# OpenVisualCloud/SVT-VP9

Hardware: AMD Instinct MI355X
Metric: hot-path frames/sec (+ Mpixels/sec): block-level DSP path (picture analysis + ME + inter prediction from reconstructed references + DCT/quant/recon + deblock + reference padding), 3840x2160p60 yuv420p enc-mode 8; no mode decision, no entropy coding -- not encoded frames (higher is better)
Workload: dtype u8

## Files before the change

### include/svtvp9_hip.h

```cpp
#ifndef SVTVP9_HIP_H
#define SVTVP9_HIP_H

#include <stddef.h>
#include <stdint.h>

#ifdef __cplusplus
extern "C" {
#endif

typedef enum svt_hip_status {
    SVT_HIP_OK                 = 0,
    SVT_HIP_ERR_BAD_PARAMETER  = -1,
    SVT_HIP_ERR_NO_RESOURCES   = -2,
    SVT_HIP_ERR_DEVICE         = -3,
    SVT_HIP_ERR_UNSUPPORTED    = -4
} svt_hip_status;

typedef struct svt_hip_ctx svt_hip_ctx;


#define SVT_ME_PU_COUNT 85
#define SVT_SB_SIZE 64

typedef struct svt_plane {
// ... 52 lines not shown

typedef struct svt_me_pu_result {
    int16_t         x_mv_l0, y_mv_l0, x_mv_l1, y_mv_l1;
    svt_me_dist_dir distortion_direction[3];
    uint8_t         total_me_candidate_index;
    uint8_t         pad_[7];
} svt_me_pu_result;

int32_t svt_hip_sb_count(int32_t pic_width, int32_t pic_height);

int32_t svt_hip_input_resolution(int32_t pic_width, int32_t pic_height);

typedef struct svt_me_picture_config {
    int32_t pic_width, pic_height;
    int32_t enc_mode;
    int32_t tune;
    int32_t frame_rate;
    int32_t num_ref_lists;
    int32_t temporal_layer_index;
    int32_t hierarchical_levels;
    int32_t is_used_as_reference;
    int32_t same_ref_poc;
    int32_t rate_control_mode;
} svt_me_picture_config;

int32_t svt_hip_me_params_derive(svt_me_params *p, const svt_me_picture_config *cfg);

int32_t svt_hip_me_params_preset(svt_me_params *p, int32_t pic_width, int32_t pic_height, int32_t enc_mode,
                                 int32_t tune, int32_t num_ref_lists, int32_t temporal_layer_index,
                                 int32_t hierarchical_levels);

int32_t svt_hip_me_kernel_instance(const svt_me_params *p);
int32_t svt_hip_me_last_instance(const svt_hip_ctx *ctx);
int32_t svt_hip_me_lds_bytes(const svt_me_params *p, int32_t compact);
int32_t svt_hip_ctx_set_intra_workgroups(svt_hip_ctx *ctx, int32_t n);
int32_t svt_hip_ctx_warm(svt_hip_ctx *ctx);
int32_t svt_hip_ctx_warm_scratch(svt_hip_ctx *ctx, int32_t scratch_bytes);
int32_t svt_hip_me_params_same_launch(const svt_me_params *a, const svt_me_params *b);

int32_t svt_hip_ctx_create(svt_hip_ctx **ctx, int32_t device_ordinal);
int32_t svt_hip_ctx_create_on_stream(svt_hip_ctx **ctx, int32_t device_ordinal, void *hip_stream);
int32_t svt_hip_ctx_create_cu_mask(svt_hip_ctx **ctx, int32_t device, const uint32_t *cu_mask, int32_t mask_words);
void *svt_hip_ctx_stream(svt_hip_ctx *ctx);
void    svt_hip_ctx_destroy(svt_hip_ctx *ctx);
int32_t svt_hip_ctx_synchronize(svt_hip_ctx *ctx);
const char *svt_hip_last_error(void);
float   svt_hip_last_kernel_ms(svt_hip_ctx *ctx);

int32_t svt_hip_mem_alloc(svt_hip_ctx *ctx, size_t bytes, void **d_ptr);
void    svt_hip_mem_free(svt_hip_ctx *ctx, void *d_ptr);
int32_t svt_hip_mem_upload_2d(svt_hip_ctx *ctx, void *d_dst, size_t dst_stride, const void *src, size_t src_stride, size_t width_bytes,
                              size_t rows);
int32_t svt_hip_mem_download(svt_hip_ctx *ctx, void *dst, const void *d_src, size_t bytes);
int32_t svt_hip_mem_upload_2d_async(svt_hip_ctx *ctx, void *d_dst, size_t dst_stride, const void *src, size_t src_stride, size_t width_bytes,
                                    size_t rows);
int32_t svt_hip_mem_upload_planes_async(svt_hip_ctx *ctx, int32_t n_planes, void *const *d_dst, const size_t *dst_stride, const void *const *src,
                                        const size_t *src_stride, const size_t *width_bytes, const size_t *rows);
int32_t svt_hip_mem_upload_2d_direct(svt_hip_ctx *ctx, void *d_dst, size_t dst_stride, const void *src, size_t src_stride, size_t width_bytes,
                                     size_t rows);
int32_t svt_hip_mem_upload_wait(svt_hip_ctx *ctx);
void    svt_hip_host_unregister_all(void);
void    svt_hip_host_registry_retain(void);
void    svt_hip_host_registry_release(void);
int32_t svt_hip_ctx_marker_record(svt_hip_ctx *ctx, uint64_t *marker);
int32_t svt_hip_ctx_marker_query(svt_hip_ctx *ctx, uint64_t marker);
int32_t svt_hip_ctx_marker_wait(svt_hip_ctx *ctx, uint64_t marker);
// ... 484 lines not shown
```

### svt-vp9_amd/binding.py

```python
import ctypes as C
import os

import numpy as np

HERE = os.path.dirname(os.path.abspath(__file__))
LIB_PATH = os.environ.get("SVT_HIP_LIB") or os.path.join(HERE, "libsvtvp9_hip.so")

SVT_ME_PU_COUNT = 85


class Plane(C.Structure):
    _fields_ = [("buf", C.c_void_p), ("stride", C.c_int32), ("origin_x", C.c_int32), ("origin_y", C.c_int32),
                ("width", C.c_int32), ("height", C.c_int32)]


class PaPicture(C.Structure):
    _fields_ = [("full", Plane), ("quarter", Plane), ("sixteenth", Plane)]


class MeParams(C.Structure):
    _fields_ = [(n, C.c_uint8) for n in (
        "num_ref_lists", "temporal_layer_index", "hierarchical_levels", "enable_hme_flag",
        "enable_hme_level_0_flag", "enable_hme_level_1_flag", "enable_hme_level_2_flag", "cu8x8_mode",
        "cu16x16_mode", "same_ref_poc", "rate_control_mode", "fractional_search_method",
# ... 138 lines not shown
MODES_TABLES_DTYPE = np.dtype([("kf_y_mode_prob", "u1", (10, 10, 9)), ("kf_uv_mode_prob", "u1", (10, 9)), ("kf_partition_probs", "u1", (16, 3)), ("skip_probs", "u1", (3,))])
assert MODES_TABLES_DTYPE.itemsize == 900 + 90 + 48 + 3
MODES_BAD_GRID = 0xFFFFFFFF
MODES_UNIT_BOOLS = 48


class ModesPicture(C.Structure):
    _fields_ = [("d_lf_mi", C.c_void_p), ("d_eob_map", C.c_void_p), ("d_tok_off", C.c_void_p), ("d_bools", C.c_void_p), ("d_segments", C.c_void_p),
                ("d_n_bools", C.c_void_p), ("capacity", C.c_uint32), ("pad_", C.c_uint32)]

OIS_BLOCK_DTYPE = np.dtype([("sad", "<u4"), ("uv_sad", "<u4"), ("mode", "u1"), ("uv_mode", "u1"), ("pad", "u1", (2,))])
assert OIS_BLOCK_DTYPE.itemsize == 12
OIS_PER_SB = 340
OIS_NONE = 0xFFFFFFFF

EXPORTS = [
    "svt_hip_sb_count", "svt_hip_input_resolution", "svt_hip_me_params_derive", "svt_hip_me_params_preset", "svt_hip_ctx_create", "svt_hip_ctx_create_on_stream", "svt_hip_ctx_create_cu_mask", "svt_hip_ctx_stream",
    "svt_hip_ctx_destroy", "svt_hip_ctx_synchronize", "svt_hip_last_error", "svt_hip_last_kernel_ms",
    "svt_hip_mem_alloc", "svt_hip_mem_free", "svt_hip_mem_upload_2d", "svt_hip_mem_upload_2d_async", "svt_hip_mem_upload_planes_async", "svt_hip_mem_download", "svt_hip_mem_set",
    "svt_hip_ctx_marker_record", "svt_hip_ctx_marker_query", "svt_hip_ctx_marker_wait", "svt_hip_minigop_split",
    "svt_hip_me_picture_device", "svt_hip_me_batch_device", "svt_hip_me_batch_layers_device", "svt_hip_me_picture", "svt_hip_sad_loop_batch_device",
    "svt_hip_me_zz_sad_device", "svt_hip_me_similar_collocated", "svt_hip_me_sb_stats_device", "svt_hip_pa_prepare_batch_device", "svt_hip_pa_mean_variance_device",
    "svt_hip_quant_tables_init", "svt_hip_tq_batch_device", "svt_hip_tq_batch_dist_device", "svt_hip_tq_rd_batch_device", "svt_hip_tq_rd_batch_multi_device", "svt_hip_rate_scan4x4_table", "svt_hip_tq_batch", "svt_hip_lf_thresh_init", "svt_hip_lf_level_from_q",
    "svt_hip_lf_frame_device", "svt_hip_lf_batch_device", "svt_hip_lf_frame", "svt_hip_lf_build_masks",
    "svt_hip_inter_pred_batch_device", "svt_hip_inter_pred_frame", "svt_hip_ref_pad_batch_device", "svt_hip_coeff_rate_batch_device", "svt_hip_coeff_rate_batch",
    "svt_hip_gop_owner", "svt_hip_gop_assign", "svt_hip_minigop_reference_source", "svt_hip_device_set_create", "svt_hip_device_set_size",
    "svt_hip_device_set_ctx", "svt_hip_device_set_destroy", "svt_hip_ref_handoff_device",
    "svt_ivf_stream_header", "svt_ivf_packetize",
    "svt_hip_tq_blocks_from_grid", "svt_hip_vp9_iscan_tables", "svt_hip_vp9_qindex_from_qp", "svt_hip_vp9_dc_step", "svt_hip_vp9_ac_step",
    "svt_hip_quant_tables_for_qindex", "svt_hip_encdec_flags_derive", "svt_hip_encdec_work_create", "svt_hip_encdec_work_destroy",
    "svt_hip_encdec_batch_device", "svt_hip_encdec_intra_device", "svt_hip_md_intra_default_device", "svt_hip_encdec_work_status", "svt_hip_encdec_work_download", "svt_hip_md_default_batch_device",
    "svt_hip_md_default_picture", "svt_hip_lf_build_masks_device", "svt_hip_ctx_wait_marker", "svt_hip_host_alloc", "svt_hip_host_free",
    "svt_hip_mem_download_2d_async", "svt_hip_mem_copy_2d_device", "svt_hip_encdec_work_set_stage_hook", "svt_hip_me_params_same_launch", "svt_hip_me_kernel_instance", "svt_hip_ctx_set_intra_workgroups", "svt_hip_ctx_warm", "svt_hip_ctx_warm_scratch", "svt_hip_lf_reserve",
    "svt_hip_me_last_instance", "svt_hip_me_lds_bytes", "svt_hip_vp9_layer_qindex", "svt_hip_mem_upload_2d_direct", "svt_hip_mem_upload_wait", "svt_hip_host_unregister_all", "svt_hip_host_registry_retain", "svt_hip_host_registry_release",
    "svt_hip_intra_search_device", "svt_hip_md_intra_search_device", "svt_hip_md_intra_search_picture",
    "svt_hip_pa_noise_params_derive", "svt_hip_pa_noise_batch_device", "svt_hip_pa_histogram_batch_device", "svt_hip_pa_chroma_mean_batch_device",
    "svt_hip_vp9_scan_tables", "svt_hip_tokenize_blocks_device", "svt_hip_tokenize_blocks", "svt_hip_tokenize_blocks_host", "svt_hip_tokenize_batch_device", "svt_hip_tokenize_picture",
    "svt_hip_tokenize_capacity",
    "svt_hip_boolcode_set_tables", "svt_hip_boolcode_batch_device", "svt_hip_boolcode", "svt_hip_boolcode_host", "svt_hip_boolcode_capacity", "svt_hip_boolcode_bools_capacity",
    "svt_hip_boolcode_geometry",
    "svt_hip_modes_set_tables", "svt_hip_modes_kf_batch_device", "svt_hip_modes_kf_picture", "svt_hip_modes_segments", "svt_hip_modes_bools_capacity",
]

_lib = None


def load():
    global _lib
    if _lib is None:
        if not os.path.exists(LIB_PATH):
            raise RuntimeError(f"{LIB_PATH} not built: run `python -c 'import __graft_entry__ as g; g.build()'`")
        try:
            import torch
        except Exception:
            pass
        _lib = C.CDLL(LIB_PATH)
        _lib.svt_hip_last_error.restype = C.c_char_p
        _lib.svt_hip_ctx_stream.restype = C.c_void_p
        _lib.svt_hip_ctx_stream.argtypes = [C.c_void_p]
        _lib.svt_hip_last_kernel_ms.restype = C.c_float
        _lib.svt_hip_last_kernel_ms.argtypes = [C.c_void_p]
        _lib.svt_hip_lf_thresh_init.restype = None
        _lib.svt_hip_vp9_iscan_tables.restype = C.POINTER(C.c_int16)
        _lib.svt_hip_vp9_iscan_tables.argtypes = [C.POINTER(C.POINTER(C.c_uint32)), C.POINTER(C.c_int32)]
        _lib.svt_hip_vp9_scan_tables.restype = C.POINTER(C.c_int16)
        _lib.svt_hip_vp9_scan_tables.argtypes = [C.POINTER(C.POINTER(C.c_uint32)), C.POINTER(C.c_int32)]
        _lib.svt_hip_tokenize_capacity.restype = C.c_uint32
# ... 64 lines not shown
```

### svt-vp9_amd/csrc/me_fast.h

```cpp
#ifndef SVT_ME_FAST_H
#define SVT_ME_FAST_H
#include "me_core.h"

#ifndef SVT_HOST_EMU

constexpr bool me_fast_params_ok(uint8_t hme, uint8_t l0, uint8_t l1, uint8_t l2, uint8_t single, uint8_t method, uint8_t model, uint8_t f64,
                                 uint8_t cu16, uint8_t cu8) {
    return hme && l0 && !l1 && !l2 && single && method == SVT_SUB_SAD_SEARCH && model == 1 && !f64 && cu16 == 0 && cu8 == 1;
}

#define FME_ACC(st, s) ((uint32_t *)(st)->hme_sad + 5 * (s))
#define FME_HKEY(st, l) ((uint32_t *)(st)->hme_keys + (l))
#define FME_GATE(st) (&(st)->supel[0])
#define FME_QTAB(st) ((uint32_t *)(st)->spu)
#define FME_BTAB(st) ((uint32_t *)(st)->spu + 32)
SVT_DEV uint32_t fme_src_code(const me_ctx_t *c, int plane, int dx, int dy) {
    return plane == ME_PF ? (0x8000u | (uint32_t)(128 + ME_MUL(dy, c->L.region_stride) + dx))
                          : (uint32_t)(128 + ME_MUL(plane - 1, c->L.plane_bytes) + ME_MUL(dy, c->L.plane_stride) + dx);
}

SVT_DEV uint32_t fme_wave_sum63(uint32_t v) {
    v = svt_row_prefix_add(v, 16);
    v += (uint32_t)__builtin_amdgcn_update_dpp(0, (int)v, 0x142, 0xa, 0xf, false);
    v += (uint32_t)__builtin_amdgcn_update_dpp(0, (int)v, 0x143, 0xc, 0xf, false);
// ... 83 lines not shown
        uint32_t        lo = q[0];
        _Pragma("unroll") for (int i = 0; i < 8; i++) {
            const uint32_t hi = q[i + 1];
            acc = svt_sad4(svt_alignbyte(hi, lo, sh), sp[i], acc);
            lo = hi;
        }
    }
    acc = fme_wave_sum63(acc);
    if (tid == 63) slot[0] = acc;
}

SVT_DEV void fph_load_rect(int tid, uint8_t *dst, int dst_stride, const uint8_t *src, int src_stride, int nd, int rows) {
    const int      nu = (nd + 3) >> 2, n = nu * rows, last = 4 * nd - 16;
    const uint32_t inv = me_magics.v[nu];
    for (int t0 = tid; t0 < n; t0 += 2 * SVT_NT) {
        me_u32x4 v[2];
        int      o[2];
        _Pragma("unroll") for (int u = 0; u < 2; u++) {
            const int t = t0 + u * SVT_NT;
            o[u] = -1;
            if (t < n) {
                const int r = inv ? (int)__umulhi((uint32_t)t, inv) : t, i = t - ME_MUL(r, nu);
                const int b = 16 * i < last ? 16 * i : last;
                v[u] = me_ld128u_g(src + (uint32_t)(ME_MUL(r, src_stride) + b));
                o[u] = ME_MUL(r, dst_stride) + b;
            }
        }
        _Pragma("unroll") for (int u = 0; u < 2; u++)
            if (o[u] >= 0) {
                uint32_t *d = (uint32_t *)(dst + o[u]);
                d[0] = v[u].x; d[1] = v[u].y; d[2] = v[u].z; d[3] = v[u].w;
            }
    }
}

template <int WS> SVT_DEV void fph_hme_search(const me_ctx_t *c, int tid, int ws_rt, int sw, int nr, int y0, uint32_t *key) {
    const int      ws = WS ? WS : ws_rt, ng2 = sw >> 3, ntask = ME_MUL(ng2, nr);
    const uint32_t inv = me_magics.v[ng2];
    uint32_t       b0 = 0xffffffffu, b1 = 0xffffffffu, b2 = 0xffffffffu, b3 = 0xffffffffu;
    const uint32_t *blk = (const uint32_t *)c->st->sixteenth_sb;
    const bool tile32 = ng2 == 8;
    const int  nt = tile32 ? ((nr + 31) & ~31) * 8 : ntask;
    for (int T = tid; T < nt; T += SVT_NT) {
        int y, g;
        if (tile32) {
            const int l = T & 63, blk32 = T >> 8, wv = (T >> 6) & 3;
            y = 32 * blk32 + 4 * wv + ((l >> 3) & 1) + 2 * ((l >> 5) & 1) + 16 * ((l >> 4) & 1);
            g = 2 * (l & 7);
            if (y >= nr) continue;
        } else {
            y = (int)__umulhi((uint32_t)T, inv); g = 2 * (T - ME_MUL(y, ng2));
        }
        uint32_t o0 = (uint32_t)(c->planes - c->lds) + (uint32_t)(ME_MUL(y, ws) + 4 * g), o1 = o0 + 4, o2 = o0 + 12 * ws, o3 = o2 + 4;
        __asm__("" : "+v"(o0));
        __asm__("" : "+v"(o1));
        __asm__("" : "+v"(o2));
        __asm__("" : "+v"(o3));
        uint64_t acc0 = 0, acc1 = 0, acc2 = 0, acc3 = 0;
        _Pragma("unroll") for (int j = 0; j < 8; j++) {
            const uint8_t *wa = c->lds + (j < 6 ? o0 + 2 * j * ws : o2 + 2 * (j - 6) * ws), *wb = c->lds + (j < 6 ? o1 + 2 * j * ws : o3 + 2 * (j - 6) * ws);
            const uint64_t p0 = *(const me_u64a4 *)wa, p1 = *(const me_u64a4 *)wb, p2 = *(const me_u64a4 *)(wa + 8), p3 = *(const me_u64a4 *)(wb + 8),
                           p4 = *(const me_u64a4 *)(wa + 16);
            const uint32_t s0 = blk[4 * j], s1 = blk[4 * j + 1], s2 = blk[4 * j + 2], s3 = blk[4 * j + 3];
            uint64_t       a = (j & 1) ? acc1 : acc0, e = (j & 1) ? acc3 : acc2;
            a = svt_qsad(p0, s0, a); e = svt_qsad(p1, s0, e);
            a = svt_qsad(p1, s1, a); e = svt_qsad(p2, s1, e);
// ... 349 lines not shown
                uint32_t s[5];
                fme_center_sums(FME_ACC(st, 2 * list + 1), 2, s);
                z = s[0] << 1; hh = s[1] << 1;
            }
            if (z <= hh) { xsc = 0; ysc = 0; loaded = 0; }
        }
        FME_MARK(3);
        if (!loaded) {
            FME_SET_AREA();
            FME_LOAD_REGION();
        }
#undef FME_SET_AREA
#undef FME_LOAD_REGION
        FME_MARK(4);
        {
            uint32_t *U = (uint32_t *)c->planes;
            if (saw >= 8 && (saw & 7) == 0 && saw * sah <= 4096) {
                ME_PHASE(ph_fullpel_fused(c, tid, saw, sah, 0));
                FME_MARK(5);
                FME_MARK(6);
            } else {
                const int max_pos = c->L.scratch_bytes / (4 * ME_PU_STRIDE);
                int       rows_chunk = max_pos / saw;
                if (rows_chunk < 1) rows_chunk = 1;
                if (rows_chunk > sah) rows_chunk = sah;
                for (int y0 = 0; y0 < sah; y0 += rows_chunk) {
                    const int ny = y0 + rows_chunk <= sah ? rows_chunk : sah - y0;
                    ME_PHASE(ph_fullpel_sad8(c, tid, U, saw, y0, ny, w8));
                    ME_PHASE(ph_fullpel_sum16(c, tid, U, saw, ny, w8));
                    ME_PHASE(ph_fullpel_sum32(c, tid, U, ny * saw));
                    ME_PHASE(ph_fullpel_argmin(c, tid, U, saw, y0, ny));
                }
            }
            ME_PHASE(fph_decode_gate(c, tid, list, saw, sox, soy); ph_interp_strips(c, tid, W, H));
        }
        FME_MARK(7);
        const uint32_t gate = (uint32_t)ME_UNI(*FME_GATE(st));
        const int      en32 = (int)(gate & 1u), en16 = (int)((gate >> 1) & 1u);
        FME_MARK(8);
        FME_MARK(9);
        const int fast_bi = nlist == 2;
        if (en32 || en16 || fast_bi) ME_PHASE(fph_subpel(c, tid, list, sox, soy, en32, en16, fast_bi, pred0_regs));
        FME_MARK(10);
        FME_MARK(11);
        FME_MARK(12);
    }

    uint32_t *ow = (uint32_t *)c->planes;
    ME_PHASE(ph_output(c, tid, 0, ow));
    {
        uint32_t SVT_GLOBAL *g = SVT_AS_GLOBAL(uint32_t, c->pic->results + (size_t)c->sb_index * 85);
        for (int t = tid; t < 850; t += SVT_NT) g[t] = ow[t];
        if (c->pic->rcme && tid == 0) {
            uint32_t acc = 0;
            for (int i = 0; i < 16; i++) acc += ow[(5 + i) * 10 + 2];
            *SVT_AS_GLOBAL(uint32_t, &c->pic->rcme[c->sb_index]) = acc;
        }
    }
    FME_MARK(13);
}

#endif
#endif
```

### svt-vp9_amd/csrc/me_kernel.hip

```cpp
#include <hip/hip_runtime.h>
#include "me_core.h"
#include "me_fast.h"
#include "me_layout.h"
#include "me_spec.h"
#include "svt_ctx.h"
#include <stdio.h>
#include <stdlib.h>

extern __shared__ __align__(16) uint8_t svt_lds[];

#ifndef ME_WAVES_PER_EU
#define ME_WAVES_PER_EU 3
#endif
#ifndef ME_WAVES_PER_EU_SPEC
#define ME_WAVES_PER_EU_SPEC 5
#endif
template <int SPEC, bool FAST, bool COMPACT = false>
__device__ __forceinline__ void me_kernel_body(const me_pic_dev *__restrict__ pics, svt_me_params p, me_lds_layout L, int n_sb, int nx, int pic_w, int pic_h,
                                               int total, int chunk, unsigned long long *prof, uint32_t *redo = nullptr) {
    const int b = blockIdx.x, j = b >> 3;
    const int pic = j / chunk, sb = (b & 7) * chunk + (j - pic * chunk);
    if (sb >= n_sb || pic * n_sb >= total) return;
    if (!COMPACT && redo && !redo[pic * n_sb + sb]) return;
    me_ctx_t  c;
    c.redo = COMPACT ? redo + pic * n_sb + sb : nullptr;
    c.pic = &pics[pic];
    svt_me_params pp = p;
    pp.num_ref_lists = c.pic->num_ref_lists; pp.temporal_layer_index = c.pic->temporal_layer_index;
    pp.hierarchical_levels = c.pic->hierarchical_levels; pp.same_ref_poc = c.pic->same_ref_poc;
    L.hme_w0[0] = c.pic->hme_w0[0]; L.hme_w0[1] = c.pic->hme_w0[1]; L.hme_h0[0] = c.pic->hme_h0[0]; L.hme_h0[1] = c.pic->hme_h0[1];
    L.hme_tw0 = c.pic->hme_tw0; L.hme_th0 = c.pic->hme_th0;
    if constexpr (SPEC != 0) me_spec_apply<SPEC>(&pp);
    c.p   = &pp;
    if constexpr (SPEC != 0) {
        me_lds_layout G = L;
        me_lds_layout_geom_ex(&pp, &G, COMPACT);
        L.region_stride = G.region_stride; L.plane_stride = G.plane_stride; L.plane_bytes = G.plane_bytes; L.region_rows = G.region_rows;
        L.cand_dwords = G.cand_dwords; L.scratch_bytes = G.scratch_bytes;
        L.off_state = G.off_state; L.off_src = G.off_src; L.off_region = G.off_region; L.off_planes = G.off_planes;
        L.off_quarter = G.off_quarter; L.off_ssd = G.off_ssd; L.off_cand = G.off_cand; L.off_cand_hi = G.off_cand_hi; L.off_pred0 = G.off_pred0;
// ... 98 lines not shown
    static_assert(me_spec_fast(S), "me_fast.h does not serve this specialisation");
    return me_launch_kernel(svt_me_fast_kernel<S>, a, L);
}
template <int S> static hipError_t me_dispatch_sb(const me_launch_args &a, const me_lds_layout &L, const me_lds_layout &Lc, uint32_t *d_redo) {
    if constexpr (me_spec_has_compact(S))
        if (d_redo) {
            const hipError_t e = me_launch_kernel(svt_me_sb_kernel<S, true>, a, Lc, d_redo);
            return e != hipSuccess ? e : me_launch_kernel(svt_me_sb_kernel<S, false>, a, L, d_redo);
        }
    return me_launch_kernel(svt_me_sb_kernel<S, false>, a, L, (uint32_t *)nullptr);
}

static int32_t me_launch(svt_hip_ctx *ctx, int32_t n_pics, const svt_pa_picture *cur, const svt_pa_picture *ref0, const svt_pa_picture *ref1,
                         const svt_me_params *params_all, int params_stride, svt_me_pu_result *const *d_results, uint32_t *const *d_rcme) {
    if (!ctx || !cur || !ref0 || !params_all || !d_results || n_pics < 1) return svt_set_error(SVT_HIP_ERR_BAD_PARAMETER, "me: null argument");
    const svt_me_params *params = params_all;
    for (int i = 0; i < (params_stride ? n_pics : 1); i++) {
        const svt_me_params *q = &params_all[i];
        if (q->num_ref_lists < 1 || q->num_ref_lists > 2) return svt_set_error(SVT_HIP_ERR_BAD_PARAMETER, "me: num_ref_lists");
        if (q->num_ref_lists == 2 && !ref1) return svt_set_error(SVT_HIP_ERR_BAD_PARAMETER, "me: ref1 missing for B picture");
        if (q->hierarchical_levels > 5 || q->temporal_layer_index > 5 || q->number_hme_search_region_in_width > 2 ||
            q->number_hme_search_region_in_height > 2)
            return svt_set_error(SVT_HIP_ERR_BAD_PARAMETER, "me: parameter out of range");
        if (q->search_area_width < 1 || q->search_area_height < 1) return svt_set_error(SVT_HIP_ERR_BAD_PARAMETER, "me: empty full-pel search area");
        if (i && !me_params_same_config(params, q))
            return svt_set_error(SVT_HIP_ERR_BAD_PARAMETER, "me: the pictures of one launch may differ in num_ref_lists, temporal_layer_index, hierarchical_levels and same_ref_poc only");
    }
    me_lds_layout L;
    if (me_lds_layout_compute(params, &L)) return svt_set_error(SVT_HIP_ERR_UNSUPPORTED, "me: search area does not fit in LDS");
    const int W = cur[0].full.width, H = cur[0].full.height;
    if (W < 64 || H < 64 || (W & 7) || (H & 7)) return svt_set_error(SVT_HIP_ERR_BAD_PARAMETER, "me: picture size");
    const int nx = (W + 63) / 64, ny = (H + 63) / 64, n_sb = nx * ny;
    HIP_TRY(hipSetDevice(ctx->device));
    me_pic_dev *h = nullptr, *d = nullptr;
    if (svt_ctx_stage(ctx, sizeof(me_pic_dev) * (size_t)n_pics, (void **)&h, (void **)&d)) return svt_set_error(SVT_HIP_ERR_NO_RESOURCES, "me: descriptor buffers");
    bool fast_ok = (W & 63) == 0;
    for (int i = 0; i < n_pics; i++) {
        if (cur[i].full.width != W || cur[i].full.height != H) return svt_set_error(SVT_HIP_ERR_BAD_PARAMETER, "me: batch pictures differ in size");
        memset(&h[i], 0, sizeof h[i]);
        h[i].cur    = cur[i];
        h[i].ref[0] = ref0[i];
        if (ref1) h[i].ref[1] = ref1[i];
        h[i].results = d_results[i];
        h[i].rcme    = d_rcme ? d_rcme[i] : nullptr;
        const svt_me_params *q = &params_all[params_stride ? i : 0];
        me_lds_layout        Li;
        if (me_lds_layout_compute(q, &Li)) return svt_set_error(SVT_HIP_ERR_UNSUPPORTED, "me: search area does not fit in LDS");
        h[i].num_ref_lists = q->num_ref_lists; h[i].temporal_layer_index = q->temporal_layer_index;
        h[i].hierarchical_levels = q->hierarchical_levels; h[i].same_ref_poc = q->same_ref_poc;
        h[i].hme_w0[0] = Li.hme_w0[0]; h[i].hme_w0[1] = Li.hme_w0[1]; h[i].hme_h0[0] = Li.hme_h0[0]; h[i].hme_h0[1] = Li.hme_h0[1];
        h[i].hme_tw0 = Li.hme_tw0; h[i].hme_th0 = Li.hme_th0;
        {
            const int wbytes = Li.hme_tw0 + 16 + 3;
            int       ws = ((wbytes + 3) & ~3) + 4;
            if (((ws >> 2) & 1) == 0) ws += 4;
            const int band = Li.scratch_bytes / ws - 14;
            h[i].hme_band = (int16_t)(band > 256 ? 256 : band);
            if (band < 1 || Li.hme_tw0 > 256 || Li.hme_th0 > 256) fast_ok = false;
        }
    }
    HIP_TRY(hipMemcpyAsync(d, h, sizeof(me_pic_dev) * (size_t)n_pics, hipMemcpyHostToDevice, ctx->stream));
    const int total = n_sb * n_pics, chunk = (n_sb + 7) / 8;
    static const bool want_prof = getenv("SVT_HIP_ME_PROFILE") != nullptr;
    unsigned long long *d_prof = nullptr;
    if (want_prof) {
        d_prof = (unsigned long long *)svt_ctx_slot(ctx, 25, 32 * sizeof(unsigned long long));
        if (d_prof) HIP_TRY(hipMemsetAsync(d_prof, 0, 32 * sizeof(unsigned long long), ctx->stream));
    }
#ifdef ME_FINE_PROF
    { const char *sa = getenv("SVT_HIP_ME_STOP"); int v = sa ? atoi(sa) : -1; HIP_TRY(hipMemcpyToSymbolAsync(HIP_SYMBOL(g_me_stop_after), &v, sizeof v, 0, hipMemcpyHostToDevice, ctx->stream)); }
#endif
    static const bool no_spec = getenv("SVT_HIP_ME_GENERIC") != nullptr;
    static const bool no_fast = getenv("SVT_HIP_ME_NOFAST") != nullptr;
    const int spec = no_spec ? 0 : me_spec_match(params);
    me_lds_layout Lc = L;
    uint32_t     *d_redo = nullptr;
    if (me_spec_has_compact(spec) && (params->search_area_width & 7) == 0 && params->search_area_width <= 127 && me_lds_layout_compute_ex(params, &Lc, 1) == 0 &&
        me_lds_workgroups_per_cu(&Lc) > me_lds_workgroups_per_cu(&L)) {
        d_redo = (uint32_t *)svt_ctx_slot(ctx, 39, (size_t)total * sizeof(uint32_t));
        if (!d_redo) return svt_set_error(SVT_HIP_ERR_NO_RESOURCES, "me: redo flags");
        HIP_TRY(hipMemsetAsync(d_redo, 0, (size_t)total * sizeof(uint32_t), ctx->stream));
    }
    HIP_TRY(hipEventRecord(ctx->ev_start, ctx->stream));
    const bool           fast = fast_ok && !no_fast && me_spec_fast(spec);
    const me_launch_args a = {ctx->stream, chunk * 8 * n_pics, d, params, n_sb, nx, W, H, total, chunk, d_prof};
    switch (spec) {
    case 1: HIP_TRY(fast ? me_dispatch_fast<1>(a, L) : me_dispatch_sb<1>(a, L, Lc, d_redo)); break;
    case 2: HIP_TRY(me_dispatch_sb<2>(a, L, Lc, d_redo)); break;
    case 3: HIP_TRY(me_dispatch_sb<3>(a, L, Lc, d_redo)); break;
    case 4: HIP_TRY(me_dispatch_sb<4>(a, L, Lc, d_redo)); break;
    case 5: HIP_TRY(me_dispatch_sb<5>(a, L, Lc, d_redo)); break;
    default: HIP_TRY(me_dispatch_sb<0>(a, L, Lc, d_redo)); break;
    }
    ctx->me_instance = spec + (fast ? 100 : d_redo ? 200 : 0);
    HIP_TRY(hipGetLastError());
    HIP_TRY(hipEventRecord(ctx->ev_stop, ctx->stream));
    if (d_prof) {
        unsigned long long hp[32];
        HIP_TRY(hipMemcpyAsync(hp, d_prof, sizeof hp, hipMemcpyDeviceToHost, ctx->stream));
        HIP_TRY(hipStreamSynchronize(ctx->stream));
        static const char *nm[14] = {"init", "center_sads", "hme", "zero_check", "region_load", "fullpel_sad8", "fullpel_argmin",
                                     "keys2best", "supel_enable", "interp", "halfpel", "quarterpel", "pred0_bipred", "output"};
        unsigned long long tot = 0;
        for (int i = 0; i < 14; i++) tot += hp[i];
        fprintf(stderr, "[me-profile] tl=%d pics=%d WGs=%d avg cycles/WG=%llu :", params->temporal_layer_index, n_pics, total, tot / (unsigned long long)total);
        for (int i = 0; i < 14; i++) fprintf(stderr, " %s=%.1f%%", nm[i], 100.0 * (double)hp[i] / (double)tot);
        fprintf(stderr, " | hme_load=%.1f%% hme_search=%.1f%%", 100.0 * (double)hp[14] / (double)tot, 100.0 * (double)hp[15] / (double)tot);
        if (hp[20] | hp[21]) fprintf(stderr, " hme_plan=%.1f%% hme_finish=%.1f%% hme_other=%.1f%%", 100.0 * (double)hp[20] / (double)tot, 100.0 * (double)hp[21] / (double)tot, 100.0 * (double)hp[22] / (double)tot);
        if (hp[16] | hp[17] | hp[18] | hp[19])
            fprintf(stderr, " fine[lookup=%.1f%% qsad=%.1f%% keys=%.1f%% reduce=%.1f%%]", 100.0 * (double)hp[16] / (double)tot,
                    100.0 * (double)hp[17] / (double)tot, 100.0 * (double)hp[18] / (double)tot, 100.0 * (double)hp[19] / (double)tot);
        fprintf(stderr, "\n");
    }
    svt_ctx_stage_commit(ctx);
    ctx->timed = 1;
    return SVT_HIP_OK;
}

extern "C" int32_t svt_hip_me_kernel_instance(const svt_me_params *p) { return p ? me_spec_match(p) : -1; }
extern "C" int32_t svt_hip_me_last_instance(const svt_hip_ctx *ctx) { return ctx ? ctx->me_instance : -1; }
extern "C" int32_t svt_hip_me_lds_bytes(const svt_me_params *p, int32_t compact) {
    if (!p) return svt_set_error(SVT_HIP_ERR_BAD_PARAMETER, "me_lds_bytes: null argument");
    if (compact && ((p->search_area_width & 7) != 0 || p->search_area_width > 127)) return -1;
    me_lds_layout L;
    if (me_lds_layout_compute_ex(p, &L, compact ? 1 : 0)) return -1;
    return L.total_bytes;
}

extern "C" int32_t svt_hip_me_batch_device(svt_hip_ctx *ctx, int32_t n_pics, const svt_pa_picture *cur,
                                           const svt_pa_picture *ref0, const svt_pa_picture *ref1,
                                           const svt_me_params *params, svt_me_pu_result *const *d_results,
                                           uint32_t *const *d_rcme) {
    return me_launch(ctx, n_pics, cur, ref0, ref1, params, 0, d_results, d_rcme);
}
extern "C" int32_t svt_hip_me_batch_layers_device(svt_hip_ctx *ctx, int32_t n_pics, const svt_pa_picture *cur,
                                                  const svt_pa_picture *ref0, const svt_pa_picture *ref1,
                                                  const svt_me_params *params, svt_me_pu_result *const *d_results,
                                                  uint32_t *const *d_rcme) {
    return me_launch(ctx, n_pics, cur, ref0, ref1, params, 1, d_results, d_rcme);
}

extern "C" int32_t svt_hip_me_picture_device(svt_hip_ctx *ctx, const svt_pa_picture *cur, const svt_pa_picture *ref0,
                                             const svt_pa_picture *ref1, const svt_me_params *params,
                                             svt_me_pu_result *d_results, uint32_t *d_rcme) {
    svt_me_pu_result *r[1] = {d_results};
    uint32_t         *c[1] = {d_rcme};
    return svt_hip_me_batch_device(ctx, 1, cur, ref0, ref1, params, r, d_rcme ? c : nullptr);
}

static int upload_plane(svt_hip_ctx *ctx, const svt_plane *h, svt_plane *d, int slot) {
    const size_t bytes = (size_t)h->stride * (size_t)(h->height + 2 * h->origin_y);
    uint8_t     *dev   = (uint8_t *)svt_ctx_slot(ctx, slot, bytes + 64);
    if (!dev) return -1;
// ... 169 lines not shown
```

### svt-vp9_amd/csrc/me_types.h

```cpp
#ifndef SVT_ME_TYPES_H
#define SVT_ME_TYPES_H
#include "me_prims.h"

#define ME_SB 64
#define ME_MAX_SAD_VALUE (64 * 64 * 255)

typedef struct me_pic_dev {
    svt_pa_picture    cur, ref[2];
    svt_me_pu_result *results;
    uint32_t         *rcme;
    uint8_t           num_ref_lists, temporal_layer_index, hierarchical_levels, same_ref_poc;
    int16_t           hme_w0[2], hme_h0[2], hme_tw0, hme_th0;
    int16_t           hme_band;
} me_pic_dev;

typedef struct me_lds_layout {
    int32_t off_state;
    int32_t off_src;
    int32_t off_region;
    int32_t off_planes;
    int32_t off_quarter;
    int32_t off_ssd;
    int32_t off_cand;
    int32_t off_cand_hi;
    int32_t cand_dwords;
    int32_t off_pred0;
    int32_t region_stride, region_rows;
    int32_t plane_stride;
    int32_t plane_bytes;
    int32_t scratch_bytes;
    int32_t total_bytes;
    int32_t compact;
    int16_t hme_w0[2], hme_h0[2], hme_tw0, hme_th0;
} me_lds_layout;

#define ME_RGN_GX 4
#define ME_RGN_GY 3
#define ME_PL_G 2

#define ME_HME_MAX_WIN 16
typedef struct me_hme_win {
    int16_t  gx, gy;
    uint32_t off;
    uint16_t wstride;
    uint16_t tl, ts;
    uint16_t sw, sh;
// ... 89 lines not shown
```

### svt-vp9_amd/csrc/svt_ctx.h

```cpp
#ifndef SVT_CTX_H
#define SVT_CTX_H
#include <hip/hip_runtime.h>
#include <stdint.h>
#include <string.h>
#include "../../include/svtvp9_hip.h"

#define SVT_CTX_SLOTS 52
#define SVT_CTX_RING 64
#define SVT_CTX_UPLOAD_RING 4
#define SVT_CTX_MARKERS 1024

struct svt_hip_ctx {
    int         device;
    hipStream_t stream;
    int         owns_stream;
    hipEvent_t  ev_start, ev_stop;
    int         timed;
    int         cu_count;
    int         me_instance;
    int         intra_wgs;
    void       *ring_host[SVT_CTX_RING];
    void       *ring_dev[SVT_CTX_RING];
    size_t      ring_bytes[SVT_CTX_RING];
    hipEvent_t  ring_ev[SVT_CTX_RING];
    int         ring_used[SVT_CTX_RING];
    int         ring_own[SVT_CTX_RING];
    void       *ring_slab_host, *ring_slab_dev;
    int         ring_pos;
    void       *up_host[SVT_CTX_UPLOAD_RING];
    size_t      up_bytes[SVT_CTX_UPLOAD_RING];
    hipEvent_t  up_ev[SVT_CTX_UPLOAD_RING];
    int         up_used[SVT_CTX_UPLOAD_RING];
    int         up_pos;
    double      up_prof[3];
    long        up_prof_n;
    hipEvent_t  direct_ev;
    int         direct_pending;
    hipEvent_t  mk_ev[SVT_CTX_MARKERS];
    uint64_t    mk_next;
    hipEvent_t  ho_produced, ho_consumed;
    void       *slot[SVT_CTX_SLOTS];
    size_t      slot_bytes[SVT_CTX_SLOTS];
};

int32_t svt_set_error(int32_t code, const char *msg);
int32_t svt_set_hip_error(hipError_t e, const char *file, int line);
int     svt_ctx_stage(svt_hip_ctx *ctx, size_t bytes, void **host, void **dev);
void    svt_ctx_stage_commit(svt_hip_ctx *ctx);
void   *svt_ctx_slot(svt_hip_ctx *ctx, int slot, size_t bytes);

int32_t svt_tq_launch_device_lists(svt_hip_ctx *ctx, const uint8_t *d_src, const uint8_t *d_pred, uint8_t *const *recon_set, int n_set,
                                   const svt_tq_block *d_blocks, const int32_t cap[4], const int32_t *d_off_cnt, const svt_quant_tables *d_qtabs,
// ... 14 lines not shown
```

Measured before the change: 6820.

## Precompute half-pel reference planes once per batch and load them in ME

Adds a separate kernel that interpolates the b/h/j half-pel planes for each distinct reference frame once per ME batch, stored in a context slot. The fast ME kernel then copies precomputed plane windows into LDS instead of interpolating strips per superblock. This removes redundant interpolation when several pictures in a batch share a reference, at the cost of an extra launch, three full-size plane buffers and extra global memory traffic. The path is used only when the batch has at least two pictures and a reference is reused.

```diff
diff --git a/include/svtvp9_hip.h b/include/svtvp9_hip.h
--- a/include/svtvp9_hip.h
+++ b/include/svtvp9_hip.h
@@ -108,6 +108,9 @@
 
 int32_t svt_hip_me_kernel_instance(const svt_me_params *p);
 int32_t svt_hip_me_last_instance(const svt_hip_ctx *ctx);
+int32_t svt_hip_me_last_halfpel_refs(const svt_hip_ctx *ctx);
+int32_t svt_hip_me_halfpel_planes_device(svt_hip_ctx *ctx, int32_t n, const svt_plane *src, uint8_t *const *d_b, uint8_t *const *d_h,
+                                         uint8_t *const *d_j);
 int32_t svt_hip_me_lds_bytes(const svt_me_params *p, int32_t compact);
 int32_t svt_hip_ctx_set_intra_workgroups(svt_hip_ctx *ctx, int32_t n);
 int32_t svt_hip_ctx_warm(svt_hip_ctx *ctx);
diff --git a/svt-vp9_amd/binding.py b/svt-vp9_amd/binding.py
--- a/svt-vp9_amd/binding.py
+++ b/svt-vp9_amd/binding.py
@@ -194,7 +194,7 @@
     "svt_hip_encdec_batch_device", "svt_hip_encdec_intra_device", "svt_hip_md_intra_default_device", "svt_hip_encdec_work_status", "svt_hip_encdec_work_download", "svt_hip_md_default_batch_device",
     "svt_hip_md_default_picture", "svt_hip_lf_build_masks_device", "svt_hip_ctx_wait_marker", "svt_hip_host_alloc", "svt_hip_host_free",
     "svt_hip_mem_download_2d_async", "svt_hip_mem_copy_2d_device", "svt_hip_encdec_work_set_stage_hook", "svt_hip_me_params_same_launch", "svt_hip_me_kernel_instance", "svt_hip_ctx_set_intra_workgroups", "svt_hip_ctx_warm", "svt_hip_ctx_warm_scratch", "svt_hip_lf_reserve",
-    "svt_hip_me_last_instance", "svt_hip_me_lds_bytes", "svt_hip_vp9_layer_qindex", "svt_hip_mem_upload_2d_direct", "svt_hip_mem_upload_wait", "svt_hip_host_unregister_all", "svt_hip_host_registry_retain", "svt_hip_host_registry_release",
+    "svt_hip_me_last_instance", "svt_hip_me_last_halfpel_refs", "svt_hip_me_halfpel_planes_device", "svt_hip_me_lds_bytes", "svt_hip_vp9_layer_qindex", "svt_hip_mem_upload_2d_direct", "svt_hip_mem_upload_wait", "svt_hip_host_unregister_all", "svt_hip_host_registry_retain", "svt_hip_host_registry_release",
     "svt_hip_intra_search_device", "svt_hip_md_intra_search_device", "svt_hip_md_intra_search_picture",
     "svt_hip_pa_noise_params_derive", "svt_hip_pa_noise_batch_device", "svt_hip_pa_histogram_batch_device", "svt_hip_pa_chroma_mean_batch_device",
     "svt_hip_vp9_scan_tables", "svt_hip_tokenize_blocks_device", "svt_hip_tokenize_blocks", "svt_hip_tokenize_blocks_host", "svt_hip_tokenize_batch_device", "svt_hip_tokenize_picture",
diff --git a/svt-vp9_amd/csrc/me_fast.h b/svt-vp9_amd/csrc/me_fast.h
--- a/svt-vp9_amd/csrc/me_fast.h
+++ b/svt-vp9_amd/csrc/me_fast.h
@@ -139,6 +139,32 @@
                 d[0] = v[u].x; d[1] = v[u].y; d[2] = v[u].z; d[3] = v[u].w;
             }
     }
+}
+
+SVT_DEV void fph_load_planes(const me_ctx_t *c, int tid, const uint8_t *g, uint32_t pitch, int src_stride, int W, int H) {
+    const int      nd = (W + 2 * ME_PL_G + 3) >> 2, rows = H + 2 * ME_PL_G, nu = (nd + 3) >> 2, n = ME_MUL(nu, rows), last = 4 * nd - 16;
+    const int      ps = c->L.plane_stride, pb = c->L.plane_bytes;
+    const uint32_t inv = me_magics.v[nu];
+    for (int t = tid ^ 128; t < n; t += SVT_NT) {
+        const int      r = (int)__umulhi((uint32_t)t, inv), i = t - ME_MUL(r, nu);
+        const int      b = 16 * i < last ? 16 * i : last;
+        const uint32_t go = (uint32_t)(ME_MUL(r, src_stride) + b);
+        const me_u32x4 vb = me_ld128u_g(g + go), vh = me_ld128u_g(g + (go + pitch)), vj = me_ld128u_g(g + (go + 2 * pitch));
+        uint8_t       *d = c->planes + ME_MUL(r, ps) + b;
+        uint32_t      *d0 = (uint32_t *)d, *d1 = (uint32_t *)(d + pb), *d2 = (uint32_t *)(d + 2 * pb);
+        d0[0] = vb.x; d0[1] = vb.y; d0[2] = vb.z; d0[3] = vb.w;
+        d1[0] = vh.x; d1[1] = vh.y; d1[2] = vh.z; d1[3] = vh.w;
+        d2[0] = vj.x; d2[1] = vj.y; d2[2] = vj.z; d2[3] = vj.w;
+    }
+}
+SVT_DEV void fph_halfpel_planes(const me_ctx_t *c, int tid, int list, int sox, int soy, int W, int H) {
+    const uint8_t *g = c->pic->halfpel[list];
+    if (g) {
+        const svt_plane *rf = &c->pic->ref[list].full;
+        const int        stride = rf->stride;
+        fph_load_planes(c, tid, g + ((ptrdiff_t)(rf->origin_y + c->sb_y + soy - ME_PL_G) * stride + rf->origin_x + c->sb_x + sox - ME_PL_G),
+                        c->pic->halfpel_pitch[list], stride, W, H);
+    } else ph_interp_strips(c, tid, W, H);
 }
 
 template <int WS> SVT_DEV void fph_hme_search(const me_ctx_t *c, int tid, int ws_rt, int sw, int nr, int y0, uint32_t *key) {
@@ -554,7 +580,7 @@
                     ME_PHASE(ph_fullpel_argmin(c, tid, U, saw, y0, ny));
                 }
             }
-            ME_PHASE(fph_decode_gate(c, tid, list, saw, sox, soy); ph_interp_strips(c, tid, W, H));
+            ME_PHASE(fph_halfpel_planes(c, tid, list, sox, soy, W, H); fph_decode_gate(c, tid, list, saw, sox, soy));
         }
         FME_MARK(7);
         const uint32_t gate = (uint32_t)ME_UNI(*FME_GATE(st));
diff --git a/svt-vp9_amd/csrc/me_halfpel.h b/svt-vp9_amd/csrc/me_halfpel.h
--- /dev/null
+++ b/svt-vp9_amd/csrc/me_halfpel.h
@@ -0,0 +1,10 @@
+#ifndef SVT_ME_HALFPEL_H
+#define SVT_ME_HALFPEL_H
+#include "me_halfpel_core.h"
+#include "svt_ctx.h"
+
+#define ME_HP_ORIGIN_X 68
+#define ME_HP_ORIGIN_Y 67
+
+int32_t svt_me_halfpel_enqueue(svt_hip_ctx *ctx, const me_hp_job *d_jobs, int n, int max_cols, int max_rows);
+#endif
diff --git a/svt-vp9_amd/csrc/me_halfpel.hip b/svt-vp9_amd/csrc/me_halfpel.hip
--- /dev/null
+++ b/svt-vp9_amd/csrc/me_halfpel.hip
@@ -0,0 +1,43 @@
+#include <hip/hip_runtime.h>
+#include "me_halfpel.h"
+
+__global__ __launch_bounds__(256) void svt_me_halfpel_kernel(const me_hp_job *__restrict__ jobs) {
+    const me_hp_job jb = jobs[blockIdx.z];
+    const int       c0 = 4 * (int)(blockIdx.x * 256 + threadIdx.x), r0 = (int)blockIdx.y * HP_STRIP;
+    if (c0 >= jb.cols || r0 >= jb.rows) return;
+    hp_strip(jb, c0, r0);
+}
+
+int32_t svt_me_halfpel_enqueue(svt_hip_ctx *ctx, const me_hp_job *d_jobs, int n, int max_cols, int max_rows) {
+    const int ncol = (max_cols + 3) / 4;
+    hipLaunchKernelGGL(svt_me_halfpel_kernel, dim3((ncol + 255) / 256, (max_rows + HP_STRIP - 1) / HP_STRIP, n), dim3(256), 0, ctx->stream, d_jobs);
+    HIP_TRY(hipGetLastError());
+    return SVT_HIP_OK;
+}
+
+extern "C" int32_t svt_hip_me_halfpel_planes_device(svt_hip_ctx *ctx, int32_t n, const svt_plane *src, uint8_t *const *d_b, uint8_t *const *d_h,
+                                                    uint8_t *const *d_j) {
+    if (!ctx || !src || !d_b || !d_h || !d_j || n < 1 || n > 65535) return svt_set_error(SVT_HIP_ERR_BAD_PARAMETER, "me_halfpel: bad argument");
+    HIP_TRY(hipSetDevice(ctx->device));
+    me_hp_job *h = nullptr, *d = nullptr;
+    if (svt_ctx_stage(ctx, sizeof(me_hp_job) * (size_t)n, (void **)&h, (void **)&d)) return svt_set_error(SVT_HIP_ERR_NO_RESOURCES, "me_halfpel: descriptor buffers");
+    int max_cols = 0, max_rows = 0;
+    for (int i = 0; i < n; i++) {
+        const svt_plane *p = &src[i];
+        if (!p->buf || !d_b[i] || !d_h[i] || !d_j[i] || p->width < 1 || p->height < 1 || p->origin_x < 0 || p->origin_y < 0 ||
+            p->stride < p->width + 2 * p->origin_x)
+            return svt_set_error(SVT_HIP_ERR_BAD_PARAMETER, "me_halfpel: plane");
+        h[i].src = p->buf; h[i].b = d_b[i]; h[i].h = d_h[i]; h[i].j = d_j[i];
+        h[i].stride = p->stride; h[i].cols = p->width + 2 * p->origin_x; h[i].rows = p->height + 2 * p->origin_y;
+        if (h[i].cols > max_cols) max_cols = h[i].cols;
+        if (h[i].rows > max_rows) max_rows = h[i].rows;
+    }
+    HIP_TRY(hipMemcpyAsync(d, h, sizeof(me_hp_job) * (size_t)n, hipMemcpyHostToDevice, ctx->stream));
+    HIP_TRY(hipEventRecord(ctx->ev_start, ctx->stream));
+    const int32_t rc = svt_me_halfpel_enqueue(ctx, d, n, max_cols, max_rows);
+    if (rc) return rc;
+    HIP_TRY(hipEventRecord(ctx->ev_stop, ctx->stream));
+    svt_ctx_stage_commit(ctx);
+    ctx->timed = 1;
+    return SVT_HIP_OK;
+}
diff --git a/svt-vp9_amd/csrc/me_halfpel_core.h b/svt-vp9_amd/csrc/me_halfpel_core.h
--- /dev/null
+++ b/svt-vp9_amd/csrc/me_halfpel_core.h
@@ -0,0 +1,60 @@
+#ifndef SVT_ME_HALFPEL_CORE_H
+#define SVT_ME_HALFPEL_CORE_H
+#include "me_prims.h"
+
+typedef struct me_hp_job {
+    const uint8_t *src;
+    uint8_t       *b, *h, *j;
+    int32_t        stride, cols, rows;
+} me_hp_job;
+
+#define HP_STRIP 64
+
+#ifdef SVT_HOST_EMU
+#define HP_ST32(p, v) do { const uint32_t v_ = (v); memcpy((p), &v_, 4); } while (0)
+#else
+#define HP_ST32(p, v) (*SVT_AS_GLOBAL(me_u32_unaligned, (p)) = (v))
+#endif
+SVT_DEV uint32_t hp_ld4(const uint8_t *row, int c, int cols) {
+    if (c >= 0 && c + 4 <= cols) return me_ld32u_g(row + c);
+    uint32_t v = 0;
+    for (int k = 0; k < 4; k++)
+        if (c + k >= 0 && c + k < cols) v |= (uint32_t)row[c + k] << (8 * k);
+    return v;
+}
+SVT_DEV void hp_st4(uint8_t *row, int c, uint32_t v, int lo, int hi) {
+    if (c >= lo && c + 3 <= hi) { HP_ST32(row + c, v); return; }
+    for (int k = 0; k < 4; k++)
+        if (c + k >= lo && c + k <= hi) row[c + k] = (uint8_t)(v >> (8 * k));
+}
+
+SVT_DEV void hp_strip(const me_hp_job jb, int c0, int r0) {
+    const int       cols = jb.cols, rows = jb.rows;
+    const size_t    stride = (size_t)jb.stride;
+    if (c0 >= cols || r0 >= rows) return;
+    const int r1 = r0 + HP_STRIP < rows ? r0 + HP_STRIP : rows;
+    const int ra = r0 > 0 ? r0 - 1 : 0, rb = r1 + 1 < rows ? r1 + 1 : rows - 1, steps = rb - ra + 1;
+    uint32_t  ve[4], vo[4], be[4], bo[4];
+    _Pragma("unroll") for (int k = 0; k < 4; k++) { ve[k] = vo[k] = be[k] = bo[k] = 0; }
+    const uint8_t *sp = jb.src + (size_t)ra * stride;
+    uint8_t       *pb = jb.b + (size_t)ra * stride, *ph = jb.h + (size_t)ra * stride, *pj = jb.j + (size_t)ra * stride;
+    for (int i0 = 0; i0 < steps; i0 += 4) {
+        _Pragma("unroll") for (int u = 0; u < 4; u++) {
+            const int i = i0 + u, r = ra + i;
+            if (i >= steps) break;
+            const uint32_t a = hp_ld4(sp, c0 - 4, cols), m = hp_ld4(sp, c0, cols), e = hp_ld4(sp, c0 + 4, cols);
+            const uint32_t lo = svt_alignbyte(m, a, 2), hi = svt_alignbyte(e, m, 2);
+            const uint32_t p1 = me_pair16(hi, lo, 1), p2 = me_pair16(hi, lo, 2), p3 = me_pair16(hi, lo, 3), p4 = me_pair16(hi, lo, 4), p5 = me_pair16(hi, lo, 5);
+            const uint32_t he = me_tap4_half(p1, p2, p3, p4), ho = me_tap4_half(p2, p3, p4, p5);
+            if (r >= r0 && r < r1) hp_st4(pb, c0, me_half_join(he, ho), 1, cols - 3);
+            ve[u] = p2; vo[u] = p3; be[u] = me_half_lanes(he); bo[u] = me_half_lanes(ho);
+            if (i >= 3 && r - 2 >= r0 && r - 2 < r1) {
+                const int o = (u + 1) & 3, x = (u + 2) & 3, y = (u + 3) & 3;
+                hp_st4(ph - 2 * stride, c0, me_half_join(me_tap4_half(ve[o], ve[x], ve[y], ve[u]), me_tap4_half(vo[o], vo[x], vo[y], vo[u])), 0, cols - 1);
+                hp_st4(pj - 2 * stride, c0, me_half_join(me_tap4_half(be[o], be[x], be[y], be[u]), me_tap4_half(bo[o], bo[x], bo[y], bo[u])), 1, cols - 3);
+            }
+            sp += stride; pb += stride; ph += stride; pj += stride;
+        }
+    }
+}
+#endif
diff --git a/svt-vp9_amd/csrc/me_kernel.hip b/svt-vp9_amd/csrc/me_kernel.hip
--- a/svt-vp9_amd/csrc/me_kernel.hip
+++ b/svt-vp9_amd/csrc/me_kernel.hip
@@ -1,11 +1,13 @@
 #include <hip/hip_runtime.h>
 #include "me_core.h"
 #include "me_fast.h"
+#include "me_halfpel.h"
 #include "me_layout.h"
 #include "me_spec.h"
 #include "svt_ctx.h"
 #include <stdio.h>
 #include <stdlib.h>
+#include <vector>
 
 extern __shared__ __align__(16) uint8_t svt_lds[];
 
@@ -170,8 +172,9 @@
     if (W < 64 || H < 64 || (W & 7) || (H & 7)) return svt_set_error(SVT_HIP_ERR_BAD_PARAMETER, "me: picture size");
     const int nx = (W + 63) / 64, ny = (H + 63) / 64, n_sb = nx * ny;
     HIP_TRY(hipSetDevice(ctx->device));
-    me_pic_dev *h = nullptr, *d = nullptr;
-    if (svt_ctx_stage(ctx, sizeof(me_pic_dev) * (size_t)n_pics, (void **)&h, (void **)&d)) return svt_set_error(SVT_HIP_ERR_NO_RESOURCES, "me: descriptor buffers");
+    me_pic_dev  *h = nullptr, *d = nullptr;
+    const size_t jobs_off = (sizeof(me_pic_dev) * (size_t)n_pics + 15) & ~(size_t)15, stage_bytes = jobs_off + sizeof(me_hp_job) * 2 * (size_t)n_pics;
+    if (svt_ctx_stage(ctx, stage_bytes, (void **)&h, (void **)&d)) return svt_set_error(SVT_HIP_ERR_NO_RESOURCES, "me: descriptor buffers");
     bool fast_ok = (W & 63) == 0;
     for (int i = 0; i < n_pics; i++) {
         if (cur[i].full.width != W || cur[i].full.height != H) return svt_set_error(SVT_HIP_ERR_BAD_PARAMETER, "me: batch pictures differ in size");
@@ -197,7 +200,54 @@
             if (band < 1 || Li.hme_tw0 > 256 || Li.hme_th0 > 256) fast_ok = false;
         }
     }
-    HIP_TRY(hipMemcpyAsync(d, h, sizeof(me_pic_dev) * (size_t)n_pics, hipMemcpyHostToDevice, ctx->stream));
+    static const bool no_spec = getenv("SVT_HIP_ME_GENERIC") != nullptr;
+    static const bool no_fast = getenv("SVT_HIP_ME_NOFAST") != nullptr;
+    const int  spec = no_spec ? 0 : me_spec_match(params);
+    const bool fast = fast_ok && !no_fast && me_spec_fast(spec);
+    static const bool hp_in_kernel = [] { const char *e = getenv("SVT_HIP_ME_HALFPEL"); return e && !strcmp(e, "kernel"); }();
+    me_hp_job *hj = (me_hp_job *)((uint8_t *)h + jobs_off);
+    int        n_hp = 0, hp_cols = 0, hp_rows = 0;
+    if (fast && !hp_in_kernel) {
+        std::vector<const svt_plane *> refs;
+        std::vector<int>               ref_of((size_t)n_pics * 2, -1);
+        std::vector<size_t>            off;
+        size_t                         bytes = 0;
+        int                            uses = 0;
+        bool                           ok = true;
+        for (int i = 0; i < n_pics && ok; i++)
+            for (int l = 0; l < h[i].num_ref_lists; l++) {
+                const svt_plane *r = &(l ? ref1 : ref0)[i].full;
+                size_t           k = 0;
+                while (k < refs.size() && !(refs[k]->buf == r->buf && refs[k]->stride == r->stride && refs[k]->origin_x == r->origin_x &&
+                                            refs[k]->origin_y == r->origin_y && refs[k]->width == r->width && refs[k]->height == r->height)) k++;
+                if (k == refs.size()) {
+                    if (!r->buf || r->width != W || r->height != H || r->origin_x < ME_HP_ORIGIN_X || r->origin_y < ME_HP_ORIGIN_Y || r->stride < W + 2 * r->origin_x) { ok = false; break; }
+                    refs.push_back(r);
+                    off.push_back(bytes);
+                    bytes += 3 * (((size_t)r->stride * (size_t)(r->height + 2 * r->origin_y) + 255) & ~(size_t)255);
+                }
+                ref_of[(size_t)i * 2 + l] = (int)k;
+                uses++;
+            }
+        uint8_t *planes = ok && n_pics >= 2 && (size_t)uses > refs.size() ? (uint8_t *)svt_ctx_slot(ctx, 52, bytes) : nullptr;
+        if (planes) {
+            n_hp = (int)refs.size();
+            for (int k = 0; k < n_hp; k++) {
+                const svt_plane *r = refs[k];
+                const size_t     pb = (k + 1 < n_hp ? off[k + 1] - off[k] : bytes - off[k]) / 3;
+                hj[k].src = r->buf; hj[k].b = planes + off[k]; hj[k].h = hj[k].b + pb; hj[k].j = hj[k].h + pb;
+                hj[k].stride = r->stride; hj[k].cols = r->width + 2 * r->origin_x; hj[k].rows = r->height + 2 * r->origin_y;
+                if (hj[k].cols > hp_cols) hp_cols = hj[k].cols;
+                if (hj[k].rows > hp_rows) hp_rows = hj[k].rows;
+            }
+            for (int i = 0; i < n_pics; i++)
+                for (int l = 0; l < h[i].num_ref_lists; l++) {
+                    const me_hp_job *jb = &hj[ref_of[(size_t)i * 2 + l]];
+                    h[i].halfpel[l] = jb->b; h[i].halfpel_pitch[l] = (uint32_t)(jb->h - jb->b);
+                }
+        }
+    }
+    HIP_TRY(hipMemcpyAsync(d, h, n_hp ? jobs_off + sizeof(me_hp_job) * (size_t)n_hp : sizeof(me_pic_dev) * (size_t)n_pics, hipMemcpyHostToDevice, ctx->stream));
     const int total = n_sb * n_pics, chunk = (n_sb + 7) / 8;
     static const bool want_prof = getenv("SVT_HIP_ME_PROFILE") != nullptr;
     unsigned long long *d_prof = nullptr;
@@ -208,9 +258,6 @@
 #ifdef ME_FINE_PROF
     { const char *sa = getenv("SVT_HIP_ME_STOP"); int v = sa ? atoi(sa) : -1; HIP_TRY(hipMemcpyToSymbolAsync(HIP_SYMBOL(g_me_stop_after), &v, sizeof v, 0, hipMemcpyHostToDevice, ctx->stream)); }
 #endif
-    static const bool no_spec = getenv("SVT_HIP_ME_GENERIC") != nullptr;
-    static const bool no_fast = getenv("SVT_HIP_ME_NOFAST") != nullptr;
-    const int spec = no_spec ? 0 : me_spec_match(params);
     me_lds_layout Lc = L;
     uint32_t     *d_redo = nullptr;
     if (me_spec_has_compact(spec) && (params->search_area_width & 7) == 0 && params->search_area_width <= 127 && me_lds_layout_compute_ex(params, &Lc, 1) == 0 &&
@@ -220,7 +267,10 @@
         HIP_TRY(hipMemsetAsync(d_redo, 0, (size_t)total * sizeof(uint32_t), ctx->stream));
     }
     HIP_TRY(hipEventRecord(ctx->ev_start, ctx->stream));
-    const bool           fast = fast_ok && !no_fast && me_spec_fast(spec);
+    if (n_hp) {
+        const int32_t rc = svt_me_halfpel_enqueue(ctx, (const me_hp_job *)((const uint8_t *)d + jobs_off), n_hp, hp_cols, hp_rows);
+        if (rc) return rc;
+    }
     const me_launch_args a = {ctx->stream, chunk * 8 * n_pics, d, params, n_sb, nx, W, H, total, chunk, d_prof};
     switch (spec) {
     case 1: HIP_TRY(fast ? me_dispatch_fast<1>(a, L) : me_dispatch_sb<1>(a, L, Lc, d_redo)); break;
@@ -231,6 +281,7 @@
     default: HIP_TRY(me_dispatch_sb<0>(a, L, Lc, d_redo)); break;
     }
     ctx->me_instance = spec + (fast ? 100 : d_redo ? 200 : 0);
+    ctx->me_halfpel_refs = n_hp;
     HIP_TRY(hipGetLastError());
     HIP_TRY(hipEventRecord(ctx->ev_stop, ctx->stream));
     if (d_prof) {
@@ -257,6 +308,7 @@
 
 extern "C" int32_t svt_hip_me_kernel_instance(const svt_me_params *p) { return p ? me_spec_match(p) : -1; }
 extern "C" int32_t svt_hip_me_last_instance(const svt_hip_ctx *ctx) { return ctx ? ctx->me_instance : -1; }
+extern "C" int32_t svt_hip_me_last_halfpel_refs(const svt_hip_ctx *ctx) { return ctx ? ctx->me_halfpel_refs : -1; }
 extern "C" int32_t svt_hip_me_lds_bytes(const svt_me_params *p, int32_t compact) {
     if (!p) return svt_set_error(SVT_HIP_ERR_BAD_PARAMETER, "me_lds_bytes: null argument");
     if (compact && ((p->search_area_width & 7) != 0 || p->search_area_width > 127)) return -1;
diff --git a/svt-vp9_amd/csrc/me_types.h b/svt-vp9_amd/csrc/me_types.h
--- a/svt-vp9_amd/csrc/me_types.h
+++ b/svt-vp9_amd/csrc/me_types.h
@@ -12,6 +12,8 @@
     uint8_t           num_ref_lists, temporal_layer_index, hierarchical_levels, same_ref_poc;
     int16_t           hme_w0[2], hme_h0[2], hme_tw0, hme_th0;
     int16_t           hme_band;
+    const uint8_t    *halfpel[2];
+    uint32_t          halfpel_pitch[2];
 } me_pic_dev;
 
 typedef struct me_lds_layout {
diff --git a/svt-vp9_amd/csrc/svt_ctx.h b/svt-vp9_amd/csrc/svt_ctx.h
--- a/svt-vp9_amd/csrc/svt_ctx.h
+++ b/svt-vp9_amd/csrc/svt_ctx.h
@@ -5,7 +5,7 @@
 #include <string.h>
 #include "../../include/svtvp9_hip.h"
 
-#define SVT_CTX_SLOTS 52
+#define SVT_CTX_SLOTS 53
 #define SVT_CTX_RING 64
 #define SVT_CTX_UPLOAD_RING 4
 #define SVT_CTX_MARKERS 1024
@@ -18,6 +18,7 @@
     int         timed;
     int         cu_count;
     int         me_instance;
+    int         me_halfpel_refs;
     int         intra_wgs;
     void       *ring_host[SVT_CTX_RING];
     void       *ring_dev[SVT_CTX_RING];
```

Result: slower. 6313 (-7.4%).
